# yu45020/Text_Segmentation_Image_Inpainting

Measured on NVIDIA H100. Metric: PartialConv UNet 512x512 images/sec (fwd+bwd), higher is better.
Workload: dtype bf16

## Files before the change

include/pconv_b200.h:

```cpp
#ifndef PCONV_B200_H_
#define PCONV_B200_H_

#include <stddef.h>
#include <stdint.h>

#ifdef __cplusplus
extern "C" {
#endif

typedef void *pcb_stream_t;

enum { PCB_F32 = 0, PCB_BF16 = 1 };
enum { PCB_ACT_NONE = 0, PCB_ACT_RELU = 1, PCB_ACT_LEAKY = 2, PCB_ACT_RELU6 = 3 };
enum { PCB_MAX_PARTS = 8 };

typedef struct {
    const void    *x;
    const uint8_t *mask;
    int32_t c;
    int32_t x_cstride;
    int32_t x_up;
    int32_t mask_up;
} pcb_part;

// ... 43 lines not shown
int pcb_pconv_backward_data(const pcb_conv *c, const void *dc, int dc_cstride, const void *w_fwd, const void *w_dgrad,
                            void *const *dx, const int32_t *dx_cstride, pcb_stream_t stream);
int pcb_conv_dgrad_at_source_resolution(const pcb_conv *c);

int pcb_conv_dgrad_fuses_relu(const pcb_conv *c);
int pcb_pconv_backward_data_relu(const pcb_conv *c, const void *dc, int dc_cstride, const void *w_dgrad, void *dx, int dx_cstride,
                                 const void *relu_x, int relu_cstride, pcb_stream_t stream);

int pcb_pconv_backward_weight(const pcb_conv *c, const void *dc, int dc_cstride, float *dw, void *workspace, pcb_stream_t stream);
int pcb_pconv_backward_weight_acc(const pcb_conv *c, const void *dc, int dc_cstride, float *dw, void *workspace, pcb_stream_t stream);

int pcb_debug_pipeline_status(int *code);
enum { PCB_ROUTE_NONE = 0, PCB_ROUTE_GENERIC = 1, PCB_ROUTE_DEPTHWISE = 2, PCB_ROUTE_STEM = 3, PCB_ROUTE_K2R = 4,
       PCB_ROUTE_SMALLCO = 5, PCB_ROUTE_TMA = 6, PCB_ROUTE_TMA_S2 = 7, PCB_ROUTE_GATHER = 8 };
int pcb_debug_conv_routes(const pcb_conv *c, int32_t routes[3]);

int pcb_mask_planes_from_dense(const float *mask_nchw, int n, int c, int h, int w, uint8_t *planes, pcb_stream_t stream);
int pcb_mask_plane_to_dense(const uint8_t *plane, int n, int h, int w, int up, float *dst_nchw, int ctot, int c0, int c,
                            pcb_stream_t stream);

int pcb_bn_stats(const void *x, int dtype, long long count, int c, double *sum, double *sqsum, pcb_stream_t stream);
int pcb_bn_stats_acc(const void *x, int dtype, long long count, int c, double *sums, pcb_stream_t stream);
int pcb_bn_forward_fused(const void *x, int dtype, long long count, int c, const double *sums, const float *gamma,
                         const float *beta, float *running_mean, float *running_var, long long *num_batches_tracked,
                         float momentum, float eps, int act, float slope, const void *residual, void *y, float *coef,
                         pcb_stream_t stream);
int pcb_bn_finalize(const double *sum, const double *sqsum, long long count, int c, const float *gamma,
                    const float *beta, float *running_mean, float *running_var, long long *num_batches_tracked,
                    float momentum, float eps, int training, float *scale, float *shift, float *save_mean,
                    float *save_invstd, pcb_stream_t stream);
// ... 142 lines not shown
```

text_segmentation_image_inpainting_b200/_lib.py:

```python
import ctypes
import os
import threading

from . import build as _build

PCB_F32, PCB_BF16 = 0, 1
ACT_NONE, ACT_RELU, ACT_LEAKY, ACT_RELU6 = 0, 1, 2, 3
MAX_PARTS = 8
SEG_FOCAL, SEG_BOOTSTRAP = 0, 1
SEG_NONE, SEG_MEAN, SEG_SUM = 0, 1, 2
CLR_TRIANGULAR, CLR_TRIANGULAR2, CLR_EXP_RANGE = 0, 1, 2
ROUTES = ("none", "generic", "depthwise", "stem", "k2r", "smallco", "tma", "tma_s2", "gather")

c_int, c_ll, c_float, c_void_p, c_size_t = ctypes.c_int, ctypes.c_longlong, ctypes.c_float, ctypes.c_void_p, ctypes.c_size_t


class Part(ctypes.Structure):
    _fields_ = [("x", c_void_p), ("mask", c_void_p), ("c", ctypes.c_int32), ("x_cstride", ctypes.c_int32),
                ("x_up", ctypes.c_int32), ("mask_up", ctypes.c_int32)]


class Conv(ctypes.Structure):
    _fields_ = [(k, ctypes.c_int32) for k in
                ("n", "h", "w", "cin", "cout", "kh", "kw", "stride", "pad_h", "pad_w", "dil", "groups", "ho", "wo",
# ... 14 lines not shown
    "pcb_pconv_forward_premasked": (c_int, [ctypes.POINTER(Conv), c_void_p, c_void_p, c_void_p, c_int, c_void_p, c_void_p, c_void_p, c_void_p]),
    "pcb_conv_fuses_bn_stats": (c_int, [ctypes.POINTER(Conv)]),
    "pcb_pconv_forward_bn": (c_int, [ctypes.POINTER(Conv), c_void_p, c_void_p, c_void_p, c_int, c_void_p, c_void_p, c_void_p, c_int, c_void_p, c_void_p]),
    "pcb_conv_fuses_affine_act": (c_int, [ctypes.POINTER(Conv)]),
    "pcb_pconv_forward_affine_act": (c_int, [ctypes.POINTER(Conv), c_void_p, c_void_p, c_void_p, c_int, c_void_p, c_void_p, c_void_p, c_int,
                                             c_void_p, c_void_p, c_int, c_float, c_void_p]),
    "pcb_seg_mask_postprocess": (c_int, [c_void_p, c_int, c_int, c_int, c_int, c_int, c_int, c_int, c_int, c_int, c_void_p, c_void_p]),
    "pcb_pconv_mask_pass":(c_int, [ctypes.POINTER(Conv), c_void_p, c_void_p, c_void_p, c_void_p]),
    "pcb_pconv_renorm_backward": (c_int, [ctypes.POINTER(Conv), c_void_p, c_int, c_void_p, c_void_p, c_int, c_void_p, c_void_p]),
    "pcb_pconv_backward_data": (c_int, [ctypes.POINTER(Conv), c_void_p, c_int, c_void_p, c_void_p, ctypes.POINTER(c_void_p),
                                        ctypes.POINTER(ctypes.c_int32), c_void_p]),
    "pcb_pconv_backward_weight": (c_int, [ctypes.POINTER(Conv), c_void_p, c_int, c_void_p, c_void_p, c_void_p]),
    "pcb_pconv_backward_weight_acc": (c_int, [ctypes.POINTER(Conv), c_void_p, c_int, c_void_p, c_void_p, c_void_p]),
    "pcb_debug_pipeline_status": (c_int, [ctypes.POINTER(c_int)]),
    "pcb_debug_conv_routes": (c_int, [ctypes.POINTER(Conv), ctypes.POINTER(ctypes.c_int32)]),
    "pcb_mask_planes_from_dense": (c_int, [c_void_p, c_int, c_int, c_int, c_int, c_void_p, c_void_p]),
    "pcb_mask_plane_to_dense": (c_int, [c_void_p, c_int, c_int, c_int, c_int, c_void_p, c_int, c_int, c_int, c_void_p]),
    "pcb_bn_stats": (c_int, [c_void_p, c_int, c_ll, c_int, c_void_p, c_void_p, c_void_p]),
    "pcb_bn_stats_acc": (c_int, [c_void_p, c_int, c_ll, c_int, c_void_p, c_void_p]),
    "pcb_bn_forward_fused": (c_int, [c_void_p, c_int, c_ll, c_int, c_void_p, c_void_p, c_void_p, c_void_p, c_void_p, c_void_p,
                                     c_float, c_float, c_int, c_float, c_void_p, c_void_p, c_void_p, c_void_p]),
    "pcb_bn_act_backward_reduce_acc": (c_int, [c_void_p, c_void_p, c_int, c_ll, c_int, c_void_p, c_void_p, c_void_p, c_void_p,
                                               c_int, c_float, c_void_p, c_void_p]),
    "pcb_bn_act_backward_small": (c_int, [c_void_p, c_void_p, c_int, c_ll, c_int, c_void_p, c_int, c_float, c_void_p, c_void_p, c_void_p, c_void_p, c_void_p]),
    "pcb_bn_finalize": (c_int, [c_void_p, c_void_p, c_ll, c_int, c_void_p, c_void_p, c_void_p, c_void_p, c_void_p,
                                c_float, c_float, c_int, c_void_p, c_void_p, c_void_p, c_void_p, c_void_p]),
    "pcb_bn_act_forward": (c_int, [c_void_p, c_int, c_ll, c_int, c_void_p, c_void_p, c_int, c_float, c_void_p, c_void_p, c_void_p]),
    "pcb_bn_act_backward_reduce": (c_int, [c_void_p, c_void_p, c_int, c_ll, c_int, c_void_p, c_void_p, c_void_p, c_void_p,
                                           c_int, c_float, c_void_p, c_void_p, c_void_p]),
    "pcb_bn_act_backward_apply": (c_int, [c_void_p, c_void_p, c_int, c_ll, c_int, c_void_p, c_void_p, c_void_p, c_void_p,
# ... 109 lines not shown
```

text_segmentation_image_inpainting_b200/csrc/api.cu:

```cuda
#include <stdarg.h>
#include <string.h>

#include <atomic>

#include "pcb_common.cuh"

static thread_local char g_err[1024] = "";
static std::atomic<unsigned long long> g_launches{0};

int pcb_set_error(const char *fmt, ...) {
    va_list ap;
    va_start(ap, fmt);
    vsnprintf(g_err, sizeof(g_err), fmt, ap);
    va_end(ap);
    return 1;
}
void pcb_count_launch(int n) { g_launches.fetch_add(static_cast<unsigned long long>(n)); }

extern "C" __attribute__((visibility("default"))) const char *pcb_last_error(void) { return g_err; }
extern "C" __attribute__((visibility("default"))) int pcb_version(void) { return 1; }
extern "C" __attribute__((visibility("default"))) unsigned long long pcb_launch_count(void) { return g_launches.load(); }

static int validate(const pcb_conv *c, bool need_x) {
    PCB_CHECK(c != nullptr, "null pcb_conv");
// ... 191 lines not shown
    PCB_CHECK(code != nullptr, "null code");
    return pcb_tc_read_abort_flag(code);
}

PCB_API int pcb_debug_conv_routes(const pcb_conv *c, int32_t routes[3]) {
    PCB_CHECK(routes != nullptr, "null routes");
    if (int rc = validate(c, false)) return rc;
    const Family f = family_of(c);
    if (f == FAMILY_TC) {
        pcb_tc_routes(c, routes);
        return 0;
    }
    routes[0] = routes[1] = routes[2] = (f == FAMILY_DW) ? PCB_ROUTE_DEPTHWISE : PCB_ROUTE_GENERIC;
    return 0;
}
```

text_segmentation_image_inpainting_b200/csrc/conv_tc.cu:

```cuda
#include <cuda.h>
#include <stdlib.h>
#include <string.h>

#include <algorithm>

#include "pcb_common.cuh"
#include "pcb_ptx.cuh"
#include "pcb_tc_epi.cuh"

namespace {

__device__ __forceinline__ float warp_transpose_sum(float (&v)[32], int lane) {
#pragma unroll
    for (int off = 16, n = 32; off >= 1; off >>= 1, n >>= 1) {
        const bool upper = (lane & off) != 0;
#pragma unroll
        for (int i = 0; i < 16; ++i) {
            if (i < (n >> 1)) {
                const float send = upper ? v[i] : v[i + (n >> 1)];
                const float keep = upper ? v[i + (n >> 1)] : v[i];
                v[i] = keep + __shfl_xor_sync(0xffffffffu, send, off);
            }
        }
    }
// ... 366 lines not shown
                ptx::wgmma_wait<0>();
                ptx::wgmma_fence_regs(acc);
                if (leader) {
                    ptx::mbar_arrive(bar_empty_b + 8 * sb);
                    ptx::mbar_arrive(bar_empty_a + 8 * sa);
                }
            }
            if (dead) { stat_n0 = -1; break; }
            mma_epilogue<BLOCK_N, MODE>(P, acc, acc_stage, e, lane, m0, n0, my_stat);
        }
        if (my_stat && stat_n0 >= 0) tc_stats_flush<BLOCK_N>(P, my_stat, lane, stat_n0, R.cb, R.ce, 128);
    }
}


template <int BLOCK_N, int MODE, bool HALO>
__global__ void __maxnreg__(TMA_REGS)
pconv_tc_tma_kernel(const __grid_constant__ TcParams P, const __grid_constant__ CUtensorMap tmap_w,
                    const __grid_constant__ CUtensorMap tmap_a0, const __grid_constant__ CUtensorMap tmap_a1) {
    constexpr uint32_t B_BYTES = BLOCK_N * 128;
    extern __shared__ uint8_t smem_raw[];
    const uint32_t smem_base = align1024(ptx::smem_u32(smem_raw));
    const int S = P.stages;
    const int nB = HALO ? P.kw : 1;
    const int hx = HALO ? (P.kw - 1) * P.dil : 0;
    const uint32_t A_BYTES = static_cast<uint32_t>(BLOCK_M + hx) * 128u;
    const uint32_t A_ROOM = (A_BYTES + 1023u) & ~1023u;
    const uint32_t STAGE = A_ROOM + nB * B_BYTES;
    const uint32_t STAGE_TX = A_BYTES + nB * B_BYTES;
    const uint32_t sBar = smem_base + S * STAGE;
    const uint32_t bar_full = sBar, bar_fixed = sBar + 8 * MAX_RING, bar_empty = sBar + 16 * MAX_RING;
    const uint32_t acc_full = sBar + 24 * MAX_RING, acc_empty = acc_full + 8;
    const uint32_t s_stat_addr = sBar + TMA_BAR_BYTES;
    const uint32_t s_acc = s_stat_addr + EPI_STAT_SMEM_BYTES;
    uint8_t *smem_gen = smem_raw + (smem_base - ptx::smem_u32(smem_raw));

    const int warp = __shfl_sync(0xffffffffu, threadIdx.x >> 5, 0), lane = threadIdx.x & 31;
    const int np = (MODE == 0) ? P.nparts : 1;
    const int n_tiles = P.ncols / BLOCK_N;
    const int m_tiles = (P.m_total + BLOCK_M - 1) / BLOCK_M;
    const int num_tiles = m_tiles * n_tiles;
    const int tile0 = static_cast<int>(blockIdx.x), tstep = static_cast<int>(gridDim.x);
    auto m0_of = [&](int mt) -> int { return mt * BLOCK_M; };
    const bool fix = (MODE == 0) && P.use_fix;
    const int kwi = HALO ? 1 : P.kw;

    auto tile_active = [&](int n0) -> bool {
        if (MODE == 0) return true;
        for (int p = 0; p < P.nparts; ++p)
            if (P.parts[p].dx && n0 < P.parts[p].koff + P.parts[p].kext && n0 + BLOCK_N > P.parts[p].koff) return true;
        return false;
    };

    if (threadIdx.x == 0) {
        for (int s = 0; s < MAX_RING; ++s) {
            ptx::mbar_init(bar_full + 8 * s, 1); ptx::mbar_init(bar_fixed + 8 * s, TMA_FIX_THREADS / 32); ptx::mbar_init(bar_empty + 8 * s, 2);
        }
        ptx::mbar_init(acc_full, MMA_WARPS); ptx::mbar_init(acc_empty, EPI_WARPS);
        ptx::fence_mbar_init();
    }
    if (warp == 8 && lane == 0) { ptx::prefetch_tmap(&tmap_w); ptx::prefetch_tmap(&tmap_a0); if (np > 1) ptx::prefetch_tmap(&tmap_a1); }
    __syncthreads();

    float *s_stat = nullptr;
    int stat_n0 = -1;
    bf16 *acc_stage = reinterpret_cast<bf16 *>(smem_gen + (s_acc - smem_base));
    if (warp < MMA_WARPS) {
        ptx::setmaxnreg_inc<TMA_CONSUMER_REGS>();
        const int e = warp, g = warp >> 2;
        const bool leader = (threadIdx.x & 127) == 0;
        const uint32_t ready = fix ? bar_fixed : bar_full;
        const uint64_t desc_a0 = ptx::make_smem_desc(smem_base + g * 64 * 128, 16, 1024);
        const uint64_t desc_b0 = ptx::make_smem_desc(smem_base + A_ROOM, 16, 1024);
        const uint32_t stage16 = STAGE >> 4;
        const int shift0 = (HALO && MODE == 1) ? hx * 8 : 0;
        const int dshift = HALO ? ((MODE == 1) ? -P.dil * 8 : P.dil * 8) : 0;
        const int rows_a = P.kh * kwi;
        int nb0, nb1 = 0, kl0, kl1 = 4;
        {
            const int kext = (MODE == 0) ? P.parts[0].kext : P.dc_kext, c8 = (MODE == 0) ? P.parts[0].c8 : P.dc_c8;
            nb0 = kext / BLOCK_K; kl0 = min(4, (c8 - (nb0 - 1) * BLOCK_K + 15) >> 4);
            if (MODE == 0 && np > 1) { nb1 = P.parts[1].kext / BLOCK_K; kl1 = min(4, (P.parts[1].c8 - (nb1 - 1) * BLOCK_K + 15) >> 4); }
        }
        int s = 0;
        uint32_t ph = 0, aph = 1;
        bool dead = false;
        for (int tile = tile0; tile < num_tiles && !dead; tile += tstep) {
            const int n0 = (tile % n_tiles) * BLOCK_N;
            if (!tile_active(n0)) continue;
            const ConsRows cr = cons_rows<MODE>(P, m0_of(tile / n_tiles), e, lane);
            float acc[BLOCK_N / 2];
            zero_acc(acc);
            int held = -1;
            for (int r = 0; r < rows_a && !dead; ++r) {
#pragma unroll
                for (int p = 0; p < TC_MAX_PARTS; ++p) {
                    const int nbp = (p == 0) ? nb0 : nb1, klast = (p == 0) ? kl0 : kl1;
                    for (int cb = 0; cb < nbp; ++cb) {
                        if (!__all_sync(0xffffffffu, ptx::mbar_wait(ready + 8 * s, ph, P.abort_flag, 124))) { dead = true; break; }
                        uint64_t da = desc_a0 + static_cast<uint64_t>(s * stage16 + shift0), db = desc_b0 + static_cast<uint64_t>(s * stage16);
                        const int ksteps = (cb + 1 < nbp) ? 4 : klast;
                        ptx::wgmma_fence();
                        for (int tc = 0; tc < nB; ++tc, da += dshift, db += B_BYTES >> 4) {
                            if (ksteps == 4) {
#pragma unroll
                                for (int k = 0; k < 4; ++k) ptx::wgmma_bf16<BLOCK_N, 0, 0>(acc, da + 2 * k, db + 2 * k);
                            } else {
                                for (int k = 0; k < ksteps; ++k) ptx::wgmma_bf16<BLOCK_N, 0, 0>(acc, da + 2 * k, db + 2 * k);
                            }
                        }
                        ptx::wgmma_commit();
                        ptx::wgmma_wait<1>();
                        if (held >= 0 && leader) ptx::mbar_arrive(bar_empty + 8 * held);
                        held = s;
                        if (++s == S) { s = 0; ph ^= 1; }
                    }
                    if (dead) break;
                }
            }
            ptx::wgmma_wait<0>();
            ptx::wgmma_fence_regs(acc);
            if (held >= 0 && leader) ptx::mbar_arrive(bar_empty + 8 * held);
            if (dead) break;
            if (!tma_stage_tile<BLOCK_N, MODE>(P, acc, acc_stage, acc_full, acc_empty, aph, e, lane, n0, cr, 125)) break;
        }
    } else {
        ptx::setmaxnreg_dec<TMA_SUPPORT_REGS>();
        if (warp >= EPI_WARP0) {
            const int w = warp - EPI_WARP0;
            s_stat = (MODE == 0 && P.bn_sums != nullptr)
                         ? reinterpret_cast<float *>(smem_gen + (s_stat_addr - smem_base)) + w * EPI_STAT_SLICE : nullptr;
            auto origin = [&](int tile, int &m0, int &n0) {
                m0 = m0_of(tile / n_tiles); n0 = (tile % n_tiles) * BLOCK_N;
                if (!tile_active(n0)) n0 = -1;
            };
            tma_epilogue_warps<BLOCK_N, MODE>(P, tile0, tstep, num_tiles, origin, acc_stage, acc_full, acc_empty, s_stat, stat_n0, w, lane, 126);
            ptx::named_sync(1, EPI_WARPS * 32);
            if (s_stat != nullptr && stat_n0 >= 0) tc_stats_final<BLOCK_N>(P, s_stat - w * EPI_STAT_SLICE, w, lane, stat_n0);
        } else if (warp == 8) {
            int s = 0;
            uint32_t ph = 1;
            const int plane = (MODE == 0) ? P.ho * P.wo : P.h * P.w;
            const int pwid = (MODE == 0) ? P.wo : P.w;
            const int kext0 = (MODE == 0) ? P.parts[0].kext : P.dc_kext, kext1 = (MODE == 0 && np > 1) ? P.parts[1].kext : 0;
            const int dstep = (MODE == 0) ? P.dil : -P.dil;
            const int row_k = P.wk_row, col_k = P.wk_col;
            bool dead = false;
            for (int tile = tile0; tile < num_tiles && !dead; tile += tstep) {
                const int m0 = m0_of(tile / n_tiles), n0 = (tile % n_tiles) * BLOCK_N;
                if (!tile_active(n0)) continue;
                const int img = m0 / plane, rem = m0 - img * plane;
                const int oy = rem / pwid, ox = rem - oy * pwid;
                const int x_org = (MODE == 0) ? ox * P.stride - P.pad_w : (HALO ? ox + P.pad_w - hx : ox + P.pad_w);
                const int y_org = (MODE == 0) ? oy * P.stride - P.pad_h : oy + P.pad_h;
                int krow = P.wk_base;
                for (int tr = 0, y = y_org; tr < P.kh && !dead; ++tr, y += dstep, krow += row_k)
                    for (int ti = 0, x = x_org, kidx = krow; ti < kwi && !dead; ++ti, x += dstep, kidx = krow + ti * col_k) {
#pragma unroll
                        for (int p = 0; p < TC_MAX_PARTS; ++p) {
                            const int kext = (p == 0) ? kext0 : kext1;
                            const CUtensorMap *ma = (p == 0) ? &tmap_a0 : &tmap_a1;
                            for (int c0 = 0; c0 < kext; c0 += BLOCK_K, kidx += BLOCK_K) {
                                if (!__all_sync(0xffffffffu, ptx::mbar_wait(bar_empty + 8 * s, ph, P.abort_flag, 121))) { dead = true; break; }
                                if (ptx::elect_one()) {
                                    const uint32_t full = bar_full + 8 * s, dst = smem_base + s * STAGE;
                                    ptx::mbar_arrive_expect_tx(full, STAGE_TX);
                                    ptx::tma_load_4d(dst, ma, c0, x, y, img, full);
                                    uint32_t bdst = dst + A_ROOM;
                                    for (int tc = 0, kb = kidx; tc < nB; ++tc, kb += col_k, bdst += B_BYTES)
                                        ptx::tma_load_2d(bdst, &tmap_w, kb, n0, full);
                                }
                                __syncwarp();
                                if (++s == S) { s = 0; ph ^= 1; }
                            }
                            if (dead) break;
                        }
                    }
            }
        } else {
            if (fix) {
                constexpr int FR = HALO ? 3 : 2;
                const int t = (warp - 9) * 32 + lane;
                int s = 0;
// ... 110 lines not shown
                                    __syncwarp();
                                    if (lane == 0) ptx::mbar_arrive(bar_fixed + 8 * s);
                                    if (++s == S) { s = 0; ph ^= 1; }
                                }
                                if (dead) break;
                            }
                        }
                    }
                }
            }
        }
    }

}


constexpr int SP_MAX_ITEMS = 40;
struct SpItem { int dx, dy, wk; };
struct SpTable {
    int n_items;
    SpItem it[SP_MAX_ITEMS];
};

template <int BLOCK_N>
__global__ void __maxnreg__(TMA_REGS)
pconv_tc_sp_kernel(const __grid_constant__ TcParams P, const __grid_constant__ SpTable TB, const __grid_constant__ CUtensorMap tmap_w,
                   const __grid_constant__ CUtensorMap tmap_a) {
    constexpr uint32_t B_BYTES = BLOCK_N * 128;
    constexpr uint32_t STAGE = A_STAGE_BYTES + B_BYTES;
    extern __shared__ uint8_t smem_raw[];
// ... 877 lines not shown
}

int class_kw(const pcb_conv *c, int px) { return (c->kw - ((px + c->pad_w) & 1) + 1) / 2; }

bool tma_wgrad_ok(const pcb_conv *c, int *bw, int *bh, int *bn) {
    return !is_rowpack(c) && c->stride <= 2 && kblock_box(c->wo, c->ho, bw, bh, bn) && even_upsampled_parts(c);
}

size_t up_bytes(const pcb_conv *c, int p) {
    return (static_cast<size_t>(c->n) * c->h * c->w * rup(c->parts[p].c, 8) * 2 + 255) / 256 * 256;
}
size_t tapmask_bytes(const pcb_conv *c) {
    return (static_cast<size_t>(c->nparts) * c->n * c->ho * c->wo * sizeof(uint64_t) + 255) / 256 * 256;
}

size_t tma_fixed_smem(int block_n) {
    return 1024 + TMA_BAR_BYTES + EPI_STAT_SMEM_BYTES + bf16_stage_bytes(block_n);
}

template <int BLOCK_N, int MODE, bool HALO>
int launch_tma_n(TcParams &P, const CUtensorMap &tw, const CUtensorMap &ta0, const CUtensorMap &ta1, cudaStream_t st) {
    const int nb = HALO ? P.kw : 1;
    const size_t a_room = (static_cast<size_t>(BLOCK_M + (HALO ? (P.kw - 1) * P.dil : 0)) * 128 + 1023) / 1024 * 1024;
    const size_t stage = a_room + static_cast<size_t>(nb) * BLOCK_N * 128;
    const size_t fixed = tma_fixed_smem(BLOCK_N);
    P.stages = static_cast<int>(std::min<size_t>(MAX_RING, (MAX_SMEM - fixed) / stage));
    PCB_CHECK(P.stages >= 2, "TMA-fed conv: stage of %zu bytes does not fit twice", stage);
    const size_t smem = fixed + P.stages * stage;
    auto kern = pconv_tc_tma_kernel<BLOCK_N, MODE, HALO>;
    PCB_SMEM_OPT_IN(kern, MAX_SMEM);
    const int m_tiles = (P.m_total + BLOCK_M - 1) / BLOCK_M;
    const int num_tiles = m_tiles * (P.ncols / BLOCK_N);
    const int grid = std::min(num_tiles, pcb_num_sms());
    kern<<<grid, TMA_THREADS, smem, st>>>(P, tw, ta0, ta1);
    PCB_LAUNCH_CHECK();
    return 0;
}

template <int MODE>
int launch_tma(TcParams &P, const CUtensorMap &tw, const CUtensorMap &ta0, const CUtensorMap &ta1, int bn, bool halo, cudaStream_t st) {
    PCB_CHECK(!(halo && bn == 256), "TMA-fed conv: no 256-wide row-halo tiles");
    if (halo) {
        if (bn == 128) return launch_tma_n<128, MODE, true>(P, tw, ta0, ta1, st);
        if (bn == 64) return launch_tma_n<64, MODE, true>(P, tw, ta0, ta1, st);
        return launch_tma_n<32, MODE, true>(P, tw, ta0, ta1, st);
    }
// ... 8 lines not shown
    return 3 * stage + acc_stage_bytes(block_n) <= RING_BUDGET;
}

bool halo_ok(int kw, int dil, int bw, int bh, int bn, int block_n) {
    return bw == 128 && bh == 1 && bn == 1 && kw >= 2 && 128 + (kw - 1) * dil <= 256 && halo_stages_fit(kw, dil, block_n);
}

int pick_bn(int cols, long long m_total, bool fwd, int sms) {
    const long long m_tiles = (m_total + BLOCK_M - 1) / BLOCK_M;
    if (cols <= 32) return 32;
    auto waves = [&](int b) { return (m_tiles * (cols / b) + sms - 1) / sms; };
    if (cols % 256 == 0 && 2 * waves(256) <= waves(128) && (!fwd || waves(256) == 1)) return 256;
    int bn = (cols % 128 == 0) ? 128 : 64;
    while (bn > 32 && cols % (bn / 2) == 0 && m_tiles * (cols / bn) < sms / 2) bn /= 2;
    return bn;
}

template <int MODE>
int launch_tc(TcParams &P, const CUtensorMap &tm, int bn, cudaStream_t st) {
    return (bn == 128) ? launch_persistent<128, MODE>(P, tm, st) : launch_persistent<64, MODE>(P, tm, st);
}

struct ClassStreams { cudaStream_t aux[3]; cudaEvent_t ev_fork, ev_join[3]; bool ready; };
int class_streams(ClassStreams **out) {
    static thread_local ClassStreams cs_all[PCB_MAX_DEVICES] = {};
    ClassStreams &CS = cs_all[pcb_cur_device()];
    if (!CS.ready) {
        for (int i = 0; i < 3; ++i) {
            PCB_CUDA(cudaStreamCreateWithFlags(&CS.aux[i], cudaStreamNonBlocking));
            PCB_CUDA(cudaEventCreateWithFlags(&CS.ev_join[i], cudaEventDisableTiming));
// ... 156 lines not shown
    }
    TB.n_items = ni;
    CUtensorMap ta, tw;
    if (int rc = make_tmap_nhwc(&ta, dc, P.dc_c8, c->wo, c->ho, c->n, dc_cstride, S.bw, S.bh, S.bn, 2)) return rc;
    if (int rc = make_tmap_2d(&tw, w_sp_dg, rup(S.kext_u, 128), S.kd_sp, S.kd_sp, bn)) return rc;
    return (bn == 64) ? launch_sp_n<64>(P, TB, tw, ta, st) : launch_sp_n<32>(P, TB, tw, ta, st);
}

enum TcRoute { ROUTE_NONE, ROUTE_STEM, ROUTE_K2R, ROUTE_SMALLCO, ROUTE_TMA, ROUTE_TMA_S2, ROUTE_GATHER };

struct DirPlan {
    TcRoute route;
    int box_w, box_h, box_n;
    int bn;
    bool halo;
};

struct TcPlan {
    bool ok;
    Layout L;
    long long m_out, m_in;
    size_t fwd_elems, dg_elems;
    size_t extra_fwd_off, extra_dg_off;
    size_t sp_off;
    size_t workspace;
    size_t up_off[TC_MAX_PARTS];
    DirPlan fwd, dg, wg;
    bool fwd_tapmask, wg_tapmask;
    StemPlan stem;
    K2rPlan k2r;
// ... 51 lines not shown
    } else {
        F.route = ROUTE_GATHER;
        F.bn = L.bn_f;
        T.fwd_tapmask = true;
    }

    DirPlan &D = T.dg;
    if (k2r) D.route = ROUTE_K2R;
    else if (smallco) D.route = ROUTE_SMALLCO;
    else if (L.rowpack) D.route = ROUTE_NONE;
    else if (c->stride == 1 && tile_box(c->w, c->h, &bw, &bh, &bn)) {
        D.route = ROUTE_TMA;
        D.box_w = bw; D.box_h = bh; D.box_n = bn;
        D.bn = pick_bn(L.ktap, T.m_in, false, sms);
        D.halo = c->kh <= 8 && halo_ok(c->kw, c->dil, bw, bh, bn, D.bn);
    } else if (tma_dgrad_s2_ok(c, &bw, &bh, &bn)) {
        D.route = ROUTE_TMA_S2;
        D.box_w = bw; D.box_h = bh; D.box_n = bn;
        const long long m_class = static_cast<long long>(c->n) * (c->h / 2) * (c->w / 2);
        D.bn = pick_bn(L.ktap, m_class, false, sms);
        for (int cls = 0; cls < 4; ++cls) T.cls_halo[cls] = halo_ok(class_kw(c, cls & 1), 1, bw, bh, bn, D.bn);
        T.cls_fork = ((m_class + BLOCK_M - 1) / BLOCK_M) * (L.ktap / D.bn) < sms;
    } else {
        D.route = ROUTE_GATHER;
        D.bn = (L.ktap % 128 == 0) ? 128 : 64;
    }

    const bool wg_tma = tma_wgrad_ok(c, &bw, &bh, &bn);
    DirPlan &W = T.wg;
    if (stem) W.route = ROUTE_STEM;
// ... 56 lines not shown
}

}

bool pcb_tc_eligible(const pcb_conv *c) { return common_ok(c); }

size_t pcb_tc_workspace(const pcb_conv *c) { return tc_plan(c).workspace; }

void pcb_tc_weight_layout(const pcb_conv *c, size_t *fwd_elems, size_t *dgrad_elems) {
    const TcPlan T = tc_plan(c);
    *fwd_elems = T.fwd_elems;
    *dgrad_elems = T.dg_elems;
}

bool pcb_tc_subpixel(const pcb_conv *c) { return tc_plan(c).dg_at_source; }

void pcb_tc_routes(const pcb_conv *c, int32_t routes[3]) {
    static const int32_t code[] = {PCB_ROUTE_NONE, PCB_ROUTE_STEM, PCB_ROUTE_K2R, PCB_ROUTE_SMALLCO, PCB_ROUTE_TMA, PCB_ROUTE_TMA_S2,
                                   PCB_ROUTE_GATHER};
    const TcPlan T = tc_plan(c);
    routes[0] = code[T.fwd.route]; routes[1] = code[T.dg.route]; routes[2] = code[T.wg.route];
}

int pcb_tc_weight_prepare(const pcb_conv *c, const float *w_master, void *w_fwd, void *w_dgrad, bool zero_padding, cudaStream_t st) {
    const TcPlan T = tc_plan(c);
    const Layout &L = T.L;
    const size_t fe = T.fwd_elems, de = T.dg_elems;
    if (zero_padding) {
        PCB_CUDA(cudaMemsetAsync(w_fwd, 0, fe * 2, st));
        if (w_dgrad && de) PCB_CUDA(cudaMemsetAsync(w_dgrad, 0, de * 2, st));
// ... 108 lines not shown
    for (int p = 0; p < c->nparts; ++p) {
        P.parts[p].dx = static_cast<bf16 *>(dx[p]);
        P.parts[p].dx_cstride = dx_cstride[p];
        PCB_CHECK(!dx[p] || (dx_cstride[p] % 8 == 0 && dx_cstride[p] >= P.parts[p].c8 && (reinterpret_cast<uintptr_t>(dx[p]) & 15) == 0),
                  "tensor-core dgrad: dx[%d] must be 16-byte aligned with a channel stride that is a multiple of 8", p);
    }
    P.dc = static_cast<const bf16 *>(dc); P.dc_cstride = dc_cstride; P.dc_c8 = rup(c->cout, 8); P.dc_kext = L.cout64;
    P.relu_x = static_cast<const bf16 *>(relu_x); P.relu_cstride = relu_cstride;
    P.abort_flag = flag;
    P.ncols = L.ktap;
    CUtensorMap tm;
    if (int rc = make_tmap_2d(&tm, w_dgrad, rup(L.ktap, 128), L.kd, L.kd, D.bn)) return rc;
    if (D.route == ROUTE_TMA) {
        P.box_w = D.box_w; P.box_h = D.box_h; P.box_n = D.box_n;
        P.wk_base = 0; P.wk_col = L.cout64; P.wk_row = c->kw * L.cout64;
        CUtensorMap ta;
        if (int rc = make_tmap_nhwc(&ta, dc, P.dc_c8, c->wo, c->ho, c->n, dc_cstride, D.box_w + (D.halo ? (c->kw - 1) * c->dil : 0), D.box_h, D.box_n, 1)) return rc;
        return launch_tma<1>(P, tm, ta, ta, D.bn, D.halo, st);
    }
    if (D.route == ROUTE_TMA_S2) {
        const int hh = c->h / 2, hw = c->w / 2;
        P.box_w = D.box_w; P.box_h = D.box_h; P.box_n = D.box_n;
        const bool fork = T.cls_fork;
        ClassStreams *CS = nullptr;
        if (fork) {
            if (int rc = class_streams(&CS)) return rc;
            PCB_CUDA(cudaEventRecord(CS->ev_fork, st));
        }
        for (int cls = 0; cls < 4; ++cls) {
            TcParams Q = P;
// ... 119 lines not shown
```

text_segmentation_image_inpainting_b200/csrc/pcb_common.cuh:

```cuda
#pragma once
#include <cuda_bf16.h>
#include <cuda_runtime.h>
#include <stdint.h>
#include <stdio.h>

#include "../../include/pconv_b200.h"

int pcb_set_error(const char *fmt, ...);
void pcb_count_launch(int n = 1);

#define PCB_CHECK(cond, ...)                       \
    do {                                           \
        if (!(cond)) return pcb_set_error(__VA_ARGS__); \
    } while (0)

#define PCB_CUDA(expr)                                                                           \
    do {                                                                                         \
        cudaError_t _e = (expr);                                                                 \
        if (_e != cudaSuccess)                                                                   \
            return pcb_set_error("%s:%d: %s -> %s", __FILE__, __LINE__, #expr, cudaGetErrorString(_e)); \
    } while (0)

#define PCB_LAUNCH_CHECK()                                                                        \
    do {                                                                                         \
// ... 108 lines not shown
size_t pcb_tc_workspace(const pcb_conv *c);
void pcb_tc_weight_layout(const pcb_conv *c, size_t *fwd_elems, size_t *dgrad_elems);
int pcb_tc_weight_prepare(const pcb_conv *c, const float *w_master, void *w_fwd, void *w_dgrad, bool zero_padding, cudaStream_t st);
int pcb_tc_forward_mask_pass(const pcb_conv *c, uint64_t *tapmask, cudaStream_t st);
int pcb_tc_forward_ws(const pcb_conv *c, const void *w_fwd, const float *bias, void *y, int y_cstride, const float *msum,
                      uint64_t *tapmask, bool mask_pass_done, double *bn_sums, const pcb_ep *ep, cudaStream_t st);
bool pcb_tc_fuses_epilogue(const pcb_conv *c);
bool pcb_tc_subpixel(const pcb_conv *c);
int pcb_tc_dgrad(const pcb_conv *c, const void *dc, int dc_cstride, const void *w_dgrad, void *const *dx, const int *dx_cstride,
                 cudaStream_t st, const void *relu_x = nullptr, int relu_cstride = 0);
bool pcb_tc_dgrad_fuses_relu(const pcb_conv *c);
int pcb_tc_wgrad(const pcb_conv *c, const void *dc, int dc_cstride, float *dw, void *workspace, bool zero_dw, cudaStream_t st);
int pcb_tc_read_abort_flag(int *value);
int *pcb_tc_abort_flag();
void pcb_tc_routes(const pcb_conv *c, int32_t routes[3]);
struct pcb_smallco_layout { int ktap, koff[2], cout64; long long kf, kd; };
bool pcb_smallco_eligible(const pcb_conv *c);
int pcb_smallco_forward(const pcb_conv *c, const pcb_smallco_layout &L, const void *w_fwd, const float *bias, void *y, int y_cstride, const float *msum,
                        cudaStream_t st);
int pcb_smallco_dgrad(const pcb_conv *c, const pcb_smallco_layout &L, const void *dc, int dc_cstride, const void *w_dgrad, void *const *dx, const int *dx_cstride,
                      cudaStream_t st);
int pcb_smallco_wgrad(const pcb_conv *c, const pcb_smallco_layout &L, const void *dc, int dc_cstride, float *dw, bool zero_dw, cudaStream_t st);
struct K2rPlan {
    bool ok;
    int pu, ps;
    int cu, cs, choff_u, choff_s;
    pcb_conv sub;
    size_t sub_fe, sub_de;
    size_t fwd_extra, dg_extra;
    size_t workspace;
// ... 28 lines not shown
```

text_segmentation_image_inpainting_b200/csrc/pcb_tc_epi.cuh:

```cuda
#pragma once
#include <cuda.h>

#include "pcb_common.cuh"
#include "pcb_ptx.cuh"

namespace {

constexpr int BLOCK_M = 128;
constexpr int BLOCK_K = 64;
constexpr int A_STAGE_BYTES = BLOCK_M * 128;
constexpr int NUM_PRODUCER_THREADS = 128;
constexpr int TC_MAX_PARTS = 2;
constexpr int MMA_WARPS = 8;
constexpr int MMA_THREADS = MMA_WARPS * 32;
constexpr int acc_pitch(int block_n) { return block_n + 4; }
constexpr int acc_stage_bytes(int block_n) { return BLOCK_M * acc_pitch(block_n) * 4; }

inline int rup(int v, int m) { return (v + m - 1) / m * m; }

struct TcPart {
    const bf16 *x;
    const uint64_t *tapmask;
    const uint8_t *mask;
    bf16 *dx;
// ... 1 lines not shown
};

struct TcParams {
    int n, h, w, cin, cout, kh, kw, stride, pad_h, pad_w, dil, ho, wo;
    int m_total;
    int nparts, no_guard, rowpack;
    int ncols;
    int ring_a, ring_b;
    int ktap;
    TcPart parts[TC_MAX_PARTS];
    const float *bias; const float *msum; bf16 *y; int y_cstride;
    const bf16 *dc; int dc_cstride, dc_c8, dc_kext;
    const bf16 *relu_x; int relu_cstride;
    int *abort_flag;
    int box_w, box_h, box_n, stages, use_fix;
    int wk_base, wk_row, wk_col;
    int sub, py, px, fh, fw;
    double *bn_sums;
    int bn_c;
    const float *ep_scale, *ep_shift;
    int ep_on, ep_act;
    float ep_slope;
};

constexpr int STAT_SLICE = 256;
constexpr int STAT_SMEM_BYTES = MMA_WARPS * STAT_SLICE * 4 + 16;
constexpr int EPI_WARPS = 4;
constexpr int EPI_STAT_SLICE = 512;
constexpr int EPI_STAT_SQ = EPI_STAT_SLICE / 2;
constexpr int EPI_STAT_SMEM_BYTES = EPI_WARPS * EPI_STAT_SLICE * 4;
// ... 90 lines not shown
template <int R> __device__ __forceinline__ void zero_acc(float (&a)[R]) {
#pragma unroll
    for (int i = 0; i < R; ++i) a[i] = 0.f;
}

constexpr int MAX_RING = 8;

constexpr int EPI_WARP0 = MMA_WARPS + 4;
constexpr int TMA_THREADS = (EPI_WARP0 + EPI_WARPS) * 32;
constexpr int TMA_FIX_THREADS = 96;
constexpr int TMA_REGS = 128;
constexpr int TMA_CONSUMER_REGS = 192, TMA_SUPPORT_REGS = 64;
static_assert(TMA_THREADS == 512 && 2 * 128 * TMA_CONSUMER_REGS + 2 * 128 * TMA_SUPPORT_REGS == TMA_THREADS * TMA_REGS &&
              TMA_THREADS * TMA_REGS <= 65536, "TMA-fed fwd / dgrad register budget");

constexpr size_t TMA_BAR_BYTES = 24 * MAX_RING + 16;

template <int BLOCK_N, int MODE>
__device__ __forceinline__ void tc_epilogue_bf16(const TcParams &P, const EpiRow &er, const bf16 *srow, int lane, int n0, float *s_stat) {
    const bool stats = (MODE == 0) && (s_stat != nullptr);
#pragma unroll 1
    for (int c0 = 0; c0 < BLOCK_N; c0 += 32) {
        const int col = n0 + c0;
        bf16 *orow = nullptr;
        int nstore = 0;
        int xlocal = 0;
        float scale = 1.f;
        if (MODE == 0) {
            if (er.rvalid && col < P.y_cstride) { orow = P.y + er.mo * P.y_cstride + col; nstore = min(32, P.y_cstride - col); }
        } else {
#pragma unroll
// ... 59 lines not shown
#pragma unroll
                for (int j = 0; j < 8; ++j) {
                    const float2 f = __bfloat1622float2(ob[8 * h + j]);
                    const float a = f.x * live, b = f.y * live;
                    v[2 * j] = a * a; v[2 * j + 1] = b * b;
                }
                const float q = warp_transpose_sum16(v, lane);
                if ((lane >> 4) == h) { cs = s; cq = q; }
            }
            s_stat[c0 + lane] += cs;
            s_stat[EPI_STAT_SQ + c0 + lane] += cq;
        }
    }
}

template <int BLOCK_N, int MODE, typename TileFn>
__device__ __forceinline__ void tma_epilogue_warps(const TcParams &P, int tile0, int tstep, int num_tiles, TileFn tile_origin,
                                                   const bf16 *stage, uint32_t acc_full, uint32_t acc_empty, float *s_stat,
                                                   int &stat_n0, int w, int lane, int code) {
    const int row = w * 32 + lane;
    if (s_stat) {
        for (int i = lane; i < EPI_STAT_SLICE; i += 32) s_stat[i] = 0.f;
        __syncwarp();
    }
    uint32_t ph = 0;
    for (int tile = tile0; tile < num_tiles; tile += tstep) {
        int m0, n0;
        tile_origin(tile, m0, n0);
        if (n0 < 0) continue;
        if (s_stat && n0 != stat_n0) {
            if (stat_n0 >= 0) tc_stats_flush<BLOCK_N>(P, s_stat, lane, stat_n0, 0, BLOCK_N, EPI_STAT_SQ);
            stat_n0 = n0;
        }
        const EpiRow er = tc_epi_row<MODE>(P, m0 + row, false);
        if (!__all_sync(0xffffffffu, ptx::mbar_wait(acc_full, ph, P.abort_flag, code))) { stat_n0 = -1; return; }
        ph ^= 1;
        tc_epilogue_bf16<BLOCK_N, MODE>(P, er, stage + row * bf16_pitch(BLOCK_N), lane, n0, s_stat);
        __syncwarp();
        if (lane == 0) ptx::mbar_arrive(acc_empty);
    }
}

struct ConsRows {
    float inv[2];
    bool hole[2];
};
template <int MODE>
__device__ __forceinline__ ConsRows cons_rows(const TcParams &P, int m0, int e, int lane) {
    ConsRows cr;
#pragma unroll
    for (int h = 0; h < 2; ++h) {
        cr.inv[h] = 0.f; cr.hole[h] = false;
        if (MODE == 0) {
            const EpiRow er = tc_epi_row<0>(P, m0 + 64 * (e >> 2) + 16 * (e & 3) + (lane >> 2) + 8 * h);
// ... 57 lines not shown
```

Baseline: 1158.

## Use 256-pixel M tiles for halo data-gradient TMA conv with shared B loads

Adds a TWO-segment variant of the TMA-fed conv kernel for the data-gradient path (halo, N=64). Each tile covers two 128-row M segments that share one weight (B) stage, giving two accumulators per consumer warpgroup, a second A TMA load per stage, and double-buffered accumulator barriers and staging for the epilogue. The aim is to halve weight smem traffic per output and amortise per-tile overhead. In exchange it uses more registers and smem per stage, which means fewer pipeline stages and fewer tiles for load balancing. Debug entry points to query tile sizes and cap tile_m are also added.

Result: no change. 1165, median of 6 (+0.6%).

```diff
diff --git a/include/pconv_b200.h b/include/pconv_b200.h
--- a/include/pconv_b200.h
+++ b/include/pconv_b200.h
@@ -81,6 +81,8 @@
 enum { PCB_ROUTE_NONE = 0, PCB_ROUTE_GENERIC = 1, PCB_ROUTE_DEPTHWISE = 2, PCB_ROUTE_STEM = 3, PCB_ROUTE_K2R = 4,
        PCB_ROUTE_SMALLCO = 5, PCB_ROUTE_TMA = 6, PCB_ROUTE_TMA_S2 = 7, PCB_ROUTE_GATHER = 8 };
 int pcb_debug_conv_routes(const pcb_conv *c, int32_t routes[3]);
+int pcb_debug_conv_tiles(const pcb_conv *c, int32_t tiles[6]);
+int pcb_debug_set_max_tile_m(int tile_m);
 
 int pcb_mask_planes_from_dense(const float *mask_nchw, int n, int c, int h, int w, uint8_t *planes, pcb_stream_t stream);
 int pcb_mask_plane_to_dense(const uint8_t *plane, int n, int h, int w, int up, float *dst_nchw, int ctot, int c0, int c,
diff --git a/text_segmentation_image_inpainting_b200/_lib.py b/text_segmentation_image_inpainting_b200/_lib.py
--- a/text_segmentation_image_inpainting_b200/_lib.py
+++ b/text_segmentation_image_inpainting_b200/_lib.py
@@ -52,6 +52,8 @@
     "pcb_pconv_backward_weight_acc": (c_int, [ctypes.POINTER(Conv), c_void_p, c_int, c_void_p, c_void_p, c_void_p]),
     "pcb_debug_pipeline_status": (c_int, [ctypes.POINTER(c_int)]),
     "pcb_debug_conv_routes": (c_int, [ctypes.POINTER(Conv), ctypes.POINTER(ctypes.c_int32)]),
+    "pcb_debug_conv_tiles": (c_int, [ctypes.POINTER(Conv), ctypes.POINTER(ctypes.c_int32)]),
+    "pcb_debug_set_max_tile_m": (c_int, [c_int]),
     "pcb_mask_planes_from_dense": (c_int, [c_void_p, c_int, c_int, c_int, c_int, c_void_p, c_void_p]),
     "pcb_mask_plane_to_dense": (c_int, [c_void_p, c_int, c_int, c_int, c_int, c_void_p, c_int, c_int, c_int, c_void_p]),
     "pcb_bn_stats": (c_int, [c_void_p, c_int, c_ll, c_int, c_void_p, c_void_p, c_void_p]),
diff --git a/text_segmentation_image_inpainting_b200/csrc/api.cu b/text_segmentation_image_inpainting_b200/csrc/api.cu
--- a/text_segmentation_image_inpainting_b200/csrc/api.cu
+++ b/text_segmentation_image_inpainting_b200/csrc/api.cu
@@ -229,3 +229,17 @@
     routes[0] = routes[1] = routes[2] = (f == FAMILY_DW) ? PCB_ROUTE_DEPTHWISE : PCB_ROUTE_GENERIC;
     return 0;
 }
+
+PCB_API int pcb_debug_conv_tiles(const pcb_conv *c, int32_t tiles[6]) {
+    PCB_CHECK(tiles != nullptr, "null tiles");
+    if (int rc = validate(c, false)) return rc;
+    for (int i = 0; i < 6; ++i) tiles[i] = 0;
+    if (family_of(c) == FAMILY_TC) pcb_tc_tiles(c, tiles);
+    return 0;
+}
+
+PCB_API int pcb_debug_set_max_tile_m(int tile_m) {
+    PCB_CHECK(tile_m == 128 || tile_m == 256, "max tile_m must be 128 or 256, got %d", tile_m);
+    pcb_tc_set_max_tile_m(tile_m);
+    return 0;
+}
diff --git a/text_segmentation_image_inpainting_b200/csrc/conv_tc.cu b/text_segmentation_image_inpainting_b200/csrc/conv_tc.cu
--- a/text_segmentation_image_inpainting_b200/csrc/conv_tc.cu
+++ b/text_segmentation_image_inpainting_b200/csrc/conv_tc.cu
@@ -404,20 +404,21 @@
 }
 
 
-template <int BLOCK_N, int MODE, bool HALO>
-__global__ void __maxnreg__(TMA_REGS)
-pconv_tc_tma_kernel(const __grid_constant__ TcParams P, const __grid_constant__ CUtensorMap tmap_w,
-                    const __grid_constant__ CUtensorMap tmap_a0, const __grid_constant__ CUtensorMap tmap_a1) {
+template <int BLOCK_N, int MODE, bool HALO, bool TWO>
+__device__ __forceinline__ void tma_kernel_body(const TcParams &P, const CUtensorMap &tmap_w, const CUtensorMap &tmap_a0,
+                                                const CUtensorMap &tmap_a1) {
     constexpr uint32_t B_BYTES = BLOCK_N * 128;
     extern __shared__ uint8_t smem_raw[];
     const uint32_t smem_base = align1024(ptx::smem_u32(smem_raw));
     const int S = P.stages;
+    constexpr int nseg = TWO ? 2 : 1;
+    constexpr int tile_m = nseg * BLOCK_M;
     const int nB = HALO ? P.kw : 1;
     const int hx = HALO ? (P.kw - 1) * P.dil : 0;
     const uint32_t A_BYTES = static_cast<uint32_t>(BLOCK_M + hx) * 128u;
     const uint32_t A_ROOM = (A_BYTES + 1023u) & ~1023u;
-    const uint32_t STAGE = A_ROOM + nB * B_BYTES;
-    const uint32_t STAGE_TX = A_BYTES + nB * B_BYTES;
+    const uint32_t STAGE = nseg * A_ROOM + nB * B_BYTES;
+    const uint32_t STAGE_TX = nseg * A_BYTES + nB * B_BYTES;
     const uint32_t sBar = smem_base + S * STAGE;
     const uint32_t bar_full = sBar, bar_fixed = sBar + 8 * MAX_RING, bar_empty = sBar + 16 * MAX_RING;
     const uint32_t acc_full = sBar + 24 * MAX_RING, acc_empty = acc_full + 8;
@@ -428,10 +429,10 @@
     const int warp = __shfl_sync(0xffffffffu, threadIdx.x >> 5, 0), lane = threadIdx.x & 31;
     const int np = (MODE == 0) ? P.nparts : 1;
     const int n_tiles = P.ncols / BLOCK_N;
-    const int m_tiles = (P.m_total + BLOCK_M - 1) / BLOCK_M;
+    const int m_tiles = (P.m_total + tile_m - 1) / tile_m;
     const int num_tiles = m_tiles * n_tiles;
     const int tile0 = static_cast<int>(blockIdx.x), tstep = static_cast<int>(gridDim.x);
-    auto m0_of = [&](int mt) -> int { return mt * BLOCK_M; };
+    auto m0_of = [&](int mt) -> int { return mt * tile_m; };
     const bool fix = (MODE == 0) && P.use_fix;
     const int kwi = HALO ? 1 : P.kw;
 
@@ -446,7 +447,7 @@
         for (int s = 0; s < MAX_RING; ++s) {
             ptx::mbar_init(bar_full + 8 * s, 1); ptx::mbar_init(bar_fixed + 8 * s, TMA_FIX_THREADS / 32); ptx::mbar_init(bar_empty + 8 * s, 2);
         }
-        ptx::mbar_init(acc_full, MMA_WARPS); ptx::mbar_init(acc_empty, EPI_WARPS);
+        for (int h = 0; h < 2; ++h) { ptx::mbar_init(acc_full + 16 * h, MMA_WARPS); ptx::mbar_init(acc_empty + 16 * h, EPI_WARPS); }
         ptx::fence_mbar_init();
     }
     if (warp == 8 && lane == 0) { ptx::prefetch_tmap(&tmap_w); ptx::prefetch_tmap(&tmap_a0); if (np > 1) ptx::prefetch_tmap(&tmap_a1); }
@@ -461,8 +462,8 @@
         const bool leader = (threadIdx.x & 127) == 0;
         const uint32_t ready = fix ? bar_fixed : bar_full;
         const uint64_t desc_a0 = ptx::make_smem_desc(smem_base + g * 64 * 128, 16, 1024);
-        const uint64_t desc_b0 = ptx::make_smem_desc(smem_base + A_ROOM, 16, 1024);
-        const uint32_t stage16 = STAGE >> 4;
+        const uint64_t desc_b0 = ptx::make_smem_desc(smem_base + nseg * A_ROOM, 16, 1024);
+        const uint32_t stage16 = STAGE >> 4, seg16 = A_ROOM >> 4;
         const int shift0 = (HALO && MODE == 1) ? hx * 8 : 0;
         const int dshift = HALO ? ((MODE == 1) ? -P.dil * 8 : P.dil * 8) : 0;
         const int rows_a = P.kh * kwi;
@@ -473,14 +474,18 @@
             if (MODE == 0 && np > 1) { nb1 = P.parts[1].kext / BLOCK_K; kl1 = min(4, (P.parts[1].c8 - (nb1 - 1) * BLOCK_K + 15) >> 4); }
         }
         int s = 0;
-        uint32_t ph = 0, aph = 1;
+        uint32_t ph = 0, aph[2] = {1, 1};
         bool dead = false;
         for (int tile = tile0; tile < num_tiles && !dead; tile += tstep) {
             const int n0 = (tile % n_tiles) * BLOCK_N;
             if (!tile_active(n0)) continue;
-            const ConsRows cr = cons_rows<MODE>(P, m0_of(tile / n_tiles), e, lane);
-            float acc[BLOCK_N / 2];
+            const int m0 = m0_of(tile / n_tiles);
+            const ConsRows cr = cons_rows<MODE>(P, m0, e, lane);
+            ConsRows cr1 = cr;
+            if constexpr (TWO) cr1 = cons_rows<MODE>(P, m0 + BLOCK_M, e, lane);
+            float acc[BLOCK_N / 2], acc1[TWO ? BLOCK_N / 2 : 1];
             zero_acc(acc);
+            zero_acc(acc1);
             int held = -1;
             for (int r = 0; r < rows_a && !dead; ++r) {
 #pragma unroll
@@ -494,9 +499,15 @@
                         for (int tc = 0; tc < nB; ++tc, da += dshift, db += B_BYTES >> 4) {
                             if (ksteps == 4) {
 #pragma unroll
-                                for (int k = 0; k < 4; ++k) ptx::wgmma_bf16<BLOCK_N, 0, 0>(acc, da + 2 * k, db + 2 * k);
+                                for (int k = 0; k < 4; ++k) {
+                                    ptx::wgmma_bf16<BLOCK_N, 0, 0>(acc, da + 2 * k, db + 2 * k);
+                                    if constexpr (TWO) ptx::wgmma_bf16<BLOCK_N, 0, 0>(acc1, da + seg16 + 2 * k, db + 2 * k);
+                                }
                             } else {
-                                for (int k = 0; k < ksteps; ++k) ptx::wgmma_bf16<BLOCK_N, 0, 0>(acc, da + 2 * k, db + 2 * k);
+                                for (int k = 0; k < ksteps; ++k) {
+                                    ptx::wgmma_bf16<BLOCK_N, 0, 0>(acc, da + 2 * k, db + 2 * k);
+                                    if constexpr (TWO) ptx::wgmma_bf16<BLOCK_N, 0, 0>(acc1, da + seg16 + 2 * k, db + 2 * k);
+                                }
                             }
                         }
                         ptx::wgmma_commit();
@@ -510,9 +521,14 @@
             }
             ptx::wgmma_wait<0>();
             ptx::wgmma_fence_regs(acc);
+            if constexpr (TWO) ptx::wgmma_fence_regs(acc1);
             if (held >= 0 && leader) ptx::mbar_arrive(bar_empty + 8 * held);
             if (dead) break;
-            if (!tma_stage_tile<BLOCK_N, MODE>(P, acc, acc_stage, acc_full, acc_empty, aph, e, lane, n0, cr, 125)) break;
+            if (!tma_stage_tile<BLOCK_N, MODE>(P, acc, acc_stage, acc_full, acc_empty, aph[0], e, lane, n0, cr, 125)) { dead = true; break; }
+            if constexpr (TWO) {
+                if (!tma_stage_tile<BLOCK_N, MODE>(P, acc1, acc_stage + BLOCK_M * bf16_pitch(BLOCK_N), acc_full + 16, acc_empty + 16,
+                                                   aph[1], e, lane, n0, cr1, 125)) { dead = true; break; }
+            }
         }
     } else {
         ptx::setmaxnreg_dec<TMA_SUPPORT_REGS>();
@@ -524,7 +540,10 @@
                 m0 = m0_of(tile / n_tiles); n0 = (tile % n_tiles) * BLOCK_N;
                 if (!tile_active(n0)) n0 = -1;
             };
-            tma_epilogue_warps<BLOCK_N, MODE>(P, tile0, tstep, num_tiles, origin, acc_stage, acc_full, acc_empty, s_stat, stat_n0, w, lane, 126);
+            if constexpr (TWO)
+                tma_epilogue_warps<BLOCK_N, MODE, 2>(P, tile0, tstep, num_tiles, origin, acc_stage, acc_full, acc_empty, s_stat, stat_n0, w, lane, 126);
+            else
+                tma_epilogue_warps<BLOCK_N, MODE>(P, tile0, tstep, num_tiles, origin, acc_stage, acc_full, acc_empty, s_stat, stat_n0, w, lane, 126);
             ptx::named_sync(1, EPI_WARPS * 32);
             if (s_stat != nullptr && stat_n0 >= 0) tc_stats_final<BLOCK_N>(P, s_stat - w * EPI_STAT_SLICE, w, lane, stat_n0);
         } else if (warp == 8) {
@@ -543,6 +562,13 @@
                 const int oy = rem / pwid, ox = rem - oy * pwid;
                 const int x_org = (MODE == 0) ? ox * P.stride - P.pad_w : (HALO ? ox + P.pad_w - hx : ox + P.pad_w);
                 const int y_org = (MODE == 0) ? oy * P.stride - P.pad_h : oy + P.pad_h;
+                int dx1 = 0, dy1 = 0, img1 = img;
+                if (TWO) {
+                    const int m1 = m0 + BLOCK_M;
+                    img1 = m1 / plane;
+                    const int rem1 = m1 - img1 * plane, oy1 = rem1 / pwid;
+                    dx1 = (rem1 - oy1 * pwid) - ox; dy1 = oy1 - oy;
+                }
                 int krow = P.wk_base;
                 for (int tr = 0, y = y_org; tr < P.kh && !dead; ++tr, y += dstep, krow += row_k)
                     for (int ti = 0, x = x_org, kidx = krow; ti < kwi && !dead; ++ti, x += dstep, kidx = krow + ti * col_k) {
@@ -556,7 +582,8 @@
                                     const uint32_t full = bar_full + 8 * s, dst = smem_base + s * STAGE;
                                     ptx::mbar_arrive_expect_tx(full, STAGE_TX);
                                     ptx::tma_load_4d(dst, ma, c0, x, y, img, full);
-                                    uint32_t bdst = dst + A_ROOM;
+                                    if (TWO) ptx::tma_load_4d(dst + A_ROOM, ma, c0, x + dx1, y + dy1, img1, full);
+                                    uint32_t bdst = dst + nseg * A_ROOM;
                                     for (int tc = 0, kb = kidx; tc < nB; ++tc, kb += col_k, bdst += B_BYTES)
                                         ptx::tma_load_2d(bdst, &tmap_w, kb, n0, full);
                                 }
@@ -697,6 +724,19 @@
 
 }
 
+
+template <int BLOCK_N, int MODE, bool HALO>
+__global__ void __maxnreg__(TMA_REGS)
+pconv_tc_tma_kernel(const __grid_constant__ TcParams P, const __grid_constant__ CUtensorMap tmap_w,
+                    const __grid_constant__ CUtensorMap tmap_a0, const __grid_constant__ CUtensorMap tmap_a1) {
+    if constexpr (MODE == 1 && HALO && BLOCK_N == 64) {
+        if (P.m256) {
+            tma_kernel_body<BLOCK_N, MODE, HALO, true>(P, tmap_w, tmap_a0, tmap_a1);
+            return;
+        }
+    }
+    tma_kernel_body<BLOCK_N, MODE, HALO, false>(P, tmap_w, tmap_a0, tmap_a1);
+}
 
 constexpr int SP_MAX_ITEMS = 40;
 struct SpItem { int dx, dy, wk; };
@@ -1604,22 +1644,25 @@
     return (static_cast<size_t>(c->nparts) * c->n * c->ho * c->wo * sizeof(uint64_t) + 255) / 256 * 256;
 }
 
-size_t tma_fixed_smem(int block_n) {
-    return 1024 + TMA_BAR_BYTES + EPI_STAT_SMEM_BYTES + bf16_stage_bytes(block_n);
+size_t tma_fixed_smem(int block_n, int halves = 1) {
+    return 1024 + TMA_BAR_BYTES + EPI_STAT_SMEM_BYTES + static_cast<size_t>(halves) * bf16_stage_bytes(block_n);
 }
 
 template <int BLOCK_N, int MODE, bool HALO>
 int launch_tma_n(TcParams &P, const CUtensorMap &tw, const CUtensorMap &ta0, const CUtensorMap &ta1, cudaStream_t st) {
+    PCB_CHECK(!P.m256 || (MODE == 1 && HALO && BLOCK_N == 64 && P.m_total % (2 * BLOCK_M) == 0),
+              "TMA-fed conv: 256-pixel tiles need the data gradient, row halo, N = 64 and whole tiles");
+    const int nseg = P.m256 ? 2 : 1;
     const int nb = HALO ? P.kw : 1;
     const size_t a_room = (static_cast<size_t>(BLOCK_M + (HALO ? (P.kw - 1) * P.dil : 0)) * 128 + 1023) / 1024 * 1024;
-    const size_t stage = a_room + static_cast<size_t>(nb) * BLOCK_N * 128;
-    const size_t fixed = tma_fixed_smem(BLOCK_N);
+    const size_t stage = nseg * a_room + static_cast<size_t>(nb) * BLOCK_N * 128;
+    const size_t fixed = tma_fixed_smem(BLOCK_N, nseg);
     P.stages = static_cast<int>(std::min<size_t>(MAX_RING, (MAX_SMEM - fixed) / stage));
     PCB_CHECK(P.stages >= 2, "TMA-fed conv: stage of %zu bytes does not fit twice", stage);
     const size_t smem = fixed + P.stages * stage;
     auto kern = pconv_tc_tma_kernel<BLOCK_N, MODE, HALO>;
     PCB_SMEM_OPT_IN(kern, MAX_SMEM);
-    const int m_tiles = (P.m_total + BLOCK_M - 1) / BLOCK_M;
+    const int m_tiles = (P.m_total + nseg * BLOCK_M - 1) / (nseg * BLOCK_M);
     const int num_tiles = m_tiles * (P.ncols / BLOCK_N);
     const int grid = std::min(num_tiles, pcb_num_sms());
     kern<<<grid, TMA_THREADS, smem, st>>>(P, tw, ta0, ta1);
@@ -1658,6 +1701,13 @@
     int bn = (cols % 128 == 0) ? 128 : 64;
     while (bn > 32 && cols % (bn / 2) == 0 && m_tiles * (cols / bn) < sms / 2) bn /= 2;
     return bn;
+}
+
+int g_max_tile_m = 256;
+
+bool halo_m256(bool halo, int block_n, long long m_total, int cols, int sms) {
+    if (!halo || block_n != 64 || g_max_tile_m < 256 || m_total % (2 * BLOCK_M) != 0) return false;
+    return m_total / (2 * BLOCK_M) * (cols / block_n) >= sms;
 }
 
 template <int MODE>
@@ -1844,6 +1894,7 @@
     int box_w, box_h, box_n;
     int bn;
     bool halo;
+    bool m256;
 };
 
 struct TcPlan {
@@ -1925,6 +1976,7 @@
         D.box_w = bw; D.box_h = bh; D.box_n = bn;
         D.bn = pick_bn(L.ktap, T.m_in, false, sms);
         D.halo = c->kh <= 8 && halo_ok(c->kw, c->dil, bw, bh, bn, D.bn);
+        D.m256 = halo_m256(D.halo, D.bn, T.m_in, L.ktap, sms);
     } else if (tma_dgrad_s2_ok(c, &bw, &bh, &bn)) {
         D.route = ROUTE_TMA_S2;
         D.box_w = bw; D.box_h = bh; D.box_n = bn;
@@ -2011,6 +2063,20 @@
 }
 
 bool pcb_tc_subpixel(const pcb_conv *c) { return tc_plan(c).dg_at_source; }
+
+void pcb_tc_tiles(const pcb_conv *c, int32_t tiles[6]) {
+    const TcPlan T = tc_plan(c);
+    const DirPlan *d[2] = {&T.fwd, &T.dg};
+    for (int i = 0; i < 2; ++i) {
+        const bool tma = d[i]->route == ROUTE_TMA || d[i]->route == ROUTE_TMA_S2;
+        const bool halo = d[i]->route == ROUTE_TMA_S2 ? (T.cls_halo[0] || T.cls_halo[1] || T.cls_halo[2] || T.cls_halo[3]) : d[i]->halo;
+        tiles[3 * i] = tma ? (d[i]->m256 ? 2 * BLOCK_M : BLOCK_M) : 0;
+        tiles[3 * i + 1] = tma ? d[i]->bn : 0;
+        tiles[3 * i + 2] = tma && halo;
+    }
+}
+
+void pcb_tc_set_max_tile_m(int tile_m) { g_max_tile_m = tile_m; }
 
 void pcb_tc_routes(const pcb_conv *c, int32_t routes[3]) {
     static const int32_t code[] = {PCB_ROUTE_NONE, PCB_ROUTE_STEM, PCB_ROUTE_K2R, PCB_ROUTE_SMALLCO, PCB_ROUTE_TMA, PCB_ROUTE_TMA_S2,
@@ -2149,6 +2215,7 @@
     if (D.route == ROUTE_TMA) {
         P.box_w = D.box_w; P.box_h = D.box_h; P.box_n = D.box_n;
         P.wk_base = 0; P.wk_col = L.cout64; P.wk_row = c->kw * L.cout64;
+        P.m256 = D.m256;
         CUtensorMap ta;
         if (int rc = make_tmap_nhwc(&ta, dc, P.dc_c8, c->wo, c->ho, c->n, dc_cstride, D.box_w + (D.halo ? (c->kw - 1) * c->dil : 0), D.box_h, D.box_n, 1)) return rc;
         return launch_tma<1>(P, tm, ta, ta, D.bn, D.halo, st);
diff --git a/text_segmentation_image_inpainting_b200/csrc/pcb_common.cuh b/text_segmentation_image_inpainting_b200/csrc/pcb_common.cuh
--- a/text_segmentation_image_inpainting_b200/csrc/pcb_common.cuh
+++ b/text_segmentation_image_inpainting_b200/csrc/pcb_common.cuh
@@ -146,6 +146,8 @@
 int pcb_tc_read_abort_flag(int *value);
 int *pcb_tc_abort_flag();
 void pcb_tc_routes(const pcb_conv *c, int32_t routes[3]);
+void pcb_tc_tiles(const pcb_conv *c, int32_t tiles[6]);
+void pcb_tc_set_max_tile_m(int tile_m);
 struct pcb_smallco_layout { int ktap, koff[2], cout64; long long kf, kd; };
 bool pcb_smallco_eligible(const pcb_conv *c);
 int pcb_smallco_forward(const pcb_conv *c, const pcb_smallco_layout &L, const void *w_fwd, const float *bias, void *y, int y_cstride, const float *msum,
diff --git a/text_segmentation_image_inpainting_b200/csrc/pcb_tc_epi.cuh b/text_segmentation_image_inpainting_b200/csrc/pcb_tc_epi.cuh
--- a/text_segmentation_image_inpainting_b200/csrc/pcb_tc_epi.cuh
+++ b/text_segmentation_image_inpainting_b200/csrc/pcb_tc_epi.cuh
@@ -39,6 +39,7 @@
     const bf16 *relu_x; int relu_cstride;
     int *abort_flag;
     int box_w, box_h, box_n, stages, use_fix;
+    int m256;
     int wk_base, wk_row, wk_col;
     int sub, py, px, fh, fw;
     double *bn_sums;
@@ -159,7 +160,7 @@
 static_assert(TMA_THREADS == 512 && 2 * 128 * TMA_CONSUMER_REGS + 2 * 128 * TMA_SUPPORT_REGS == TMA_THREADS * TMA_REGS &&
               TMA_THREADS * TMA_REGS <= 65536, "TMA-fed fwd / dgrad register budget");
 
-constexpr size_t TMA_BAR_BYTES = 24 * MAX_RING + 16;
+constexpr size_t TMA_BAR_BYTES = 24 * MAX_RING + 32;
 
 template <int BLOCK_N, int MODE>
 __device__ __forceinline__ void tc_epilogue_bf16(const TcParams &P, const EpiRow &er, const bf16 *srow, int lane, int n0, float *s_stat) {
@@ -249,7 +250,7 @@
     }
 }
 
-template <int BLOCK_N, int MODE, typename TileFn>
+template <int BLOCK_N, int MODE, int HALVES = 1, typename TileFn>
 __device__ __forceinline__ void tma_epilogue_warps(const TcParams &P, int tile0, int tstep, int num_tiles, TileFn tile_origin,
                                                    const bf16 *stage, uint32_t acc_full, uint32_t acc_empty, float *s_stat,
                                                    int &stat_n0, int w, int lane, int code) {
@@ -267,12 +268,15 @@
             if (stat_n0 >= 0) tc_stats_flush<BLOCK_N>(P, s_stat, lane, stat_n0, 0, BLOCK_N, EPI_STAT_SQ);
             stat_n0 = n0;
         }
-        const EpiRow er = tc_epi_row<MODE>(P, m0 + row, false);
-        if (!__all_sync(0xffffffffu, ptx::mbar_wait(acc_full, ph, P.abort_flag, code))) { stat_n0 = -1; return; }
-        ph ^= 1;
-        tc_epilogue_bf16<BLOCK_N, MODE>(P, er, stage + row * bf16_pitch(BLOCK_N), lane, n0, s_stat);
-        __syncwarp();
-        if (lane == 0) ptx::mbar_arrive(acc_empty);
+#pragma unroll
+        for (int h = 0; h < HALVES; ++h) {
+            const EpiRow er = tc_epi_row<MODE>(P, m0 + BLOCK_M * h + row, false);
+            if (!__all_sync(0xffffffffu, ptx::mbar_wait(acc_full + 16 * h, (ph >> h) & 1, P.abort_flag, code))) { stat_n0 = -1; return; }
+            ph ^= 1u << h;
+            tc_epilogue_bf16<BLOCK_N, MODE>(P, er, stage + (h * BLOCK_M + row) * bf16_pitch(BLOCK_N), lane, n0, s_stat);
+            __syncwarp();
+            if (lane == 0) ptx::mbar_arrive(acc_empty + 16 * h);
+        }
     }
 }
 
```
